# Bergvca/string_grouper

Hardware: AMD Instinct MI355X
Metric: hot-path rows/sec (the device path of match_strings: tokenise + tf-idf + postings + SpGEMM-topn, inputs resident in HBM), 663k-name self-join ntop=10 min_sim=0.8; match_strings end to end: match_strings_rows_per_s (higher is better)
Workload: dtype f32

## Files before the change

### string_grouper_amd/csrc/sg_postings.hip

```cpp
#include <stdlib.h>

#include <memory>
#include <optional>

#include "sg_internal.h"
#include "sg_scan.h"

__device__ __forceinline__ int64_t row_of_thread(int64_t g, int32_t tile_log2, int32_t n_tiles) {
    return ((g % n_tiles) << tile_log2) | (g / n_tiles);
}

template <typename T>
__global__ void __launch_bounds__(256) postings_count(const int64_t *__restrict__ indptr,
                                                      const int32_t *__restrict__ indices, int64_t n_rows,
                                                      int32_t tile_log2, int32_t n_tiles, uint32_t *seg_counts) {
    const int64_t j = row_of_thread((int64_t)blockIdx.x * blockDim.x + threadIdx.x, tile_log2, n_tiles);
    if (j >= n_rows) return;
    const int64_t lo = indptr[j], hi = indptr[j + 1];
    const uint32_t t = (uint32_t)(j >> tile_log2);
    for (int64_t p = lo; p < hi; ++p) {
        const int64_t bin = (int64_t)indices[p] * n_tiles + t;
        atomicAdd(&seg_counts[bin], 1u);
    }
}
// ... 66 lines not shown
                                                     uint32_t freq_min, float inv_norm_up, int32_t fold_log2) {
    const int64_t j = row_of_thread((int64_t)blockIdx.x * blockDim.x + threadIdx.x, tile_log2, n_tiles);
    if (j >= n_rows) return;
    const int64_t lo = indptr[j], hi = indptr[j + 1];
    const uint32_t t = (uint32_t)(j >> tile_log2);
    const uint32_t col = (uint32_t)(j & (((int64_t)1 << tile_log2) - 1));
    const float fq = out_filt ? frequent_norm_ratio<T>(indices, data, lo, hi, seg, n_tiles, freq_min, inv_norm_up) : 0.f;
    for (int64_t p = lo; p < hi; ++p) {
        const int64_t bin = (int64_t)indices[p] * n_tiles + t;
        const uint32_t pos = seg[bin] + atomicAdd(&cursor[bin], 1u);
        emit_posting<T>(out_rows, out_vals, out_filt, pos, col, data[p], fq, tile_log2, inv_norm_up, t, fold_log2);
    }
}

#define SG_POST_ROWS 4
__global__ void __launch_bounds__(1024) postings_count_lds(const int64_t *__restrict__ indptr,
                                                           const int32_t *__restrict__ indices, int64_t n_rows,
                                                           int32_t tile_log2, int32_t n_terms, int32_t split,
                                                           uint32_t *__restrict__ cnt ) {
    extern __shared__ uint32_t hist[];
    const int64_t t = blockIdx.x / split;
    const int32_t part = blockIdx.x % split;
    for (int k = threadIdx.x; k < n_terms; k += blockDim.x) hist[k] = 0;
    __syncthreads();
    const int64_t part_rows = ((int64_t)1 << tile_log2) / split;
    const int64_t j0 = (t << tile_log2) + part * part_rows;
    int64_t j1 = j0 + part_rows;
    if (j1 > n_rows) j1 = n_rows;
    const int sub = threadIdx.x & 15;
    const int64_t groups = blockDim.x >> 4;
    for (int64_t jb = j0 + (threadIdx.x >> 4) * SG_POST_ROWS; jb < j1; jb += groups * SG_POST_ROWS) {
        int64_t lo[SG_POST_ROWS], hi[SG_POST_ROWS];
#pragma unroll
        for (int r = 0; r < SG_POST_ROWS; ++r) {
            const bool valid = jb + r < j1;
            lo[r] = valid ? indptr[jb + r] : 0;
            hi[r] = valid ? indptr[jb + r + 1] : 0;
        }
        int32_t k0[SG_POST_ROWS];
#pragma unroll
        for (int r = 0; r < SG_POST_ROWS; ++r) k0[r] = lo[r] + sub < hi[r] ? indices[lo[r] + sub] : -1;
#pragma unroll
        for (int r = 0; r < SG_POST_ROWS; ++r) {
            if (k0[r] >= 0) atomicAdd(&hist[k0[r]], 1u);
            for (int64_t p = lo[r] + sub + 16; p < hi[r]; p += 16) atomicAdd(&hist[indices[p]], 1u);
        }
    }
    __syncthreads();
    uint32_t *mine = cnt + (int64_t)blockIdx.x * n_terms;
    for (int k = threadIdx.x; k < n_terms; k += blockDim.x) mine[k] = hist[k];
}

__global__ void __launch_bounds__(1024) postings_colscan_kernel(uint32_t *__restrict__ cnt, int32_t n_wgs, int32_t n_terms,
                                                                uint32_t freq_min, uint32_t *__restrict__ term_len,
                                                                uint8_t *__restrict__ is_frequent) {
    __shared__ uint32_t part_sum[16][64];
    const int kk = threadIdx.x & 63, c = threadIdx.x >> 6;
    const int64_t k = (int64_t)blockIdx.x * 64 + kk;
    const int32_t run = (n_wgs + 15) / 16;
    const int32_t w0 = c * run, w1 = min(w0 + run, n_wgs);
    uint32_t s = 0;
    if (k < n_terms)
        for (int32_t w = w0; w < w1; ++w) s += cnt[(int64_t)w * n_terms + k];
    part_sum[c][kk] = s;
    __syncthreads();
// ... 73 lines not shown
                                                          const uint32_t *__restrict__ term_start,
                                                          const uint8_t *__restrict__ is_frequent, int32_t *out_rows,
                                                          T *out_vals, uint32_t *out_filt, float inv_norm_up, int32_t fold_log2) {
    extern __shared__ uint32_t cursor[];
    uint32_t *freq_bits = cursor + n_terms;
    const int64_t t = blockIdx.x / split;
    const int32_t part = blockIdx.x % split;
    for (int k = threadIdx.x; k < (n_terms + 31) / 32; k += blockDim.x) freq_bits[k] = 0;
    const uint32_t *mine = cnt + (int64_t)blockIdx.x * n_terms;
    for (int k = threadIdx.x; k < n_terms; k += blockDim.x) cursor[k] = term_start[k] + mine[k];
    __syncthreads();
    if (out_filt)
        for (int k = threadIdx.x; k < n_terms; k += blockDim.x)
            if (is_frequent[k]) atomicOr(&freq_bits[k >> 5], 1u << (k & 31));
    __syncthreads();
    const int64_t part_rows = ((int64_t)1 << tile_log2) / split;
    const int64_t j0 = (t << tile_log2) + part * part_rows;
    int64_t j1 = j0 + part_rows;
    if (j1 > n_rows) j1 = n_rows;
    const int lane = threadIdx.x & 63, sub = lane & 15;
    (void)lane;
    const int64_t groups = blockDim.x >> 4;
    const int64_t trips = (j1 - j0 + groups * SG_POST_ROWS - 1) / (groups * SG_POST_ROWS);
    for (int64_t it = 0; it < trips; ++it) {
        const int64_t jb = j0 + (it * groups + (threadIdx.x >> 4)) * SG_POST_ROWS;
        int64_t lo[SG_POST_ROWS], hi[SG_POST_ROWS];
#pragma unroll
        for (int r = 0; r < SG_POST_ROWS; ++r) {
            const bool valid = jb + r < j1;
            lo[r] = valid ? indptr[jb + r] : 0;
            hi[r] = valid ? indptr[jb + r + 1] : 0;
        }
        int32_t k0[SG_POST_ROWS];
// ... 39 lines not shown
#endif
#if defined(SG_K3_PROBE_NO_STORE)
                if (pos == 0xFFFFFFF0u)
#endif
                emit_posting<T>(out_rows, out_vals, out_filt, pos, col, v0[r], fq[r], tile_log2, inv_norm_up, (uint32_t)t, fold_log2);
            }
            for (int64_t p = lo[r] + sub + 16; p < hi[r]; p += 16) {
                const uint32_t pos = atomicAdd(&cursor[indices[p]], 1u);
                emit_posting<T>(out_rows, out_vals, out_filt, pos, col, data[p], fq[r], tile_log2, inv_norm_up, (uint32_t)t, fold_log2);
            }
        }
    }
}

__device__ __forceinline__ uint32_t lds_get16(const uint32_t *w, uint32_t k) { return (w[k >> 1] >> ((k & 1u) << 4)) & 0xffffu; }
template <typename T>
__global__ void __launch_bounds__(1024) postings_fill_staged(const int64_t *__restrict__ indptr, const int32_t *__restrict__ indices,
                                                             const T *__restrict__ data, int64_t n_rows, int32_t tile_log2,
                                                             int32_t n_terms, int32_t split, int32_t chunk_rows, uint32_t stage_cap,
                                                             uint32_t *cnt , const uint32_t *__restrict__ term_start,
                                                             const uint8_t *__restrict__ is_frequent, uint32_t *__restrict__ out_filt,
                                                             float inv_norm_up, int32_t fold_log2) {
    extern __shared__ uint32_t lds[];
    const uint32_t w16 = ((uint32_t)n_terms + 1u) >> 1;
    uint32_t *lcnt = lds;
    uint32_t *freq_bits = lcnt + ((w16 + 3u) & ~3u);
    float *fqrow = reinterpret_cast<float *>(freq_bits + (((uint32_t)n_terms + 31u) >> 5));
    uint32_t *wave_tot = reinterpret_cast<uint32_t *>(fqrow + chunk_rows);
    uint32_t *stage = wave_tot + 32;
    const int64_t t = blockIdx.x / split;
    const int32_t part = blockIdx.x % split;
    uint32_t *mine = cnt + (int64_t)blockIdx.x * n_terms;
    for (uint32_t k = threadIdx.x; k < (((uint32_t)n_terms + 31u) >> 5); k += blockDim.x) freq_bits[k] = 0;
    __syncthreads();
    for (int k = threadIdx.x; k < n_terms; k += blockDim.x)
        if (is_frequent[k]) atomicOr(&freq_bits[k >> 5], 1u << (k & 31));
    __syncthreads();
    const int64_t part_rows = ((int64_t)1 << tile_log2) / split;
    const int64_t j0 = (t << tile_log2) + part * part_rows;
    int64_t j1 = j0 + part_rows;
    if (j1 > n_rows) j1 = n_rows;
    const int lane = threadIdx.x & 63, sub = lane & 15, wave = threadIdx.x >> 6;
    const int64_t groups = blockDim.x >> 4;
    const uint32_t last_k = (uint32_t)n_terms - 1u;
    bool any_big = false;
    for (int64_t c0 = j0; c0 < j1; c0 += chunk_rows) {
        const int64_t c1 = c0 + chunk_rows < j1 ? c0 + chunk_rows : j1;
        const int64_t e = indptr[c1] - indptr[c0];
        any_big = any_big || e > (int64_t)stage_cap || e > 65535;
    }
    for (int64_t c0 = j0; c0 < j1; c0 += chunk_rows) {
        const int64_t c1 = c0 + chunk_rows < j1 ? c0 + chunk_rows : j1;
        const int64_t trips = (c1 - c0 + groups * SG_POST_ROWS - 1) / (groups * SG_POST_ROWS);
        if (any_big) {
            for (int64_t it = 0; it < trips; ++it) {
                const int64_t jb = c0 + (it * groups + (threadIdx.x >> 4)) * SG_POST_ROWS;
#pragma unroll
                for (int r = 0; r < SG_POST_ROWS; ++r) {
                    const bool valid = jb + r < c1;
                    const int64_t lo = valid ? indptr[jb + r] : 0, hi = valid ? indptr[jb + r + 1] : 0;
                    double f2 = 0.0;
                    for (int64_t p = lo + sub; p < hi; p += 16) {
                        const int32_t k = indices[p];
                        if ((freq_bits[k >> 5] >> (k & 31)) & 1u) f2 += (double)data[p] * (double)data[p];
                    }
#pragma unroll
                    for (int d = 8; d > 0; d >>= 1) {
                        const uint64_t bits = (uint64_t)__double_as_longlong(f2);
                        const uint32_t l = (uint32_t)__shfl_xor((int)(uint32_t)bits, d, 64), h = (uint32_t)__shfl_xor((int)(uint32_t)(bits >> 32), d, 64);
                        f2 += __longlong_as_double((long long)(((uint64_t)h << 32) | l));
                    }
                    const float fq = frequent_norm_ratio_of(f2, inv_norm_up);
                    const uint32_t col = (uint32_t)(jb + r - (t << tile_log2));
                    for (int64_t p = lo + sub; p < hi; p += 16) {
                        const int32_t k = indices[p];
                        const uint32_t pos = term_start[k] + atomicAdd(&mine[k], 1u);
                        out_filt[pos] = filter_posting(col, (float)data[p], fq, tile_log2, inv_norm_up, (uint32_t)t, fold_log2);
                    }
                }
            }
            __syncthreads();
            continue;
        }
        for (uint32_t w = threadIdx.x; w < w16; w += blockDim.x) lcnt[w] = 0;
        __syncthreads();
        for (int64_t it = 0; it < trips; ++it) {
            const int64_t jb = c0 + (it * groups + (threadIdx.x >> 4)) * SG_POST_ROWS;
            int64_t lo[SG_POST_ROWS], hi[SG_POST_ROWS];
#pragma unroll
            for (int r = 0; r < SG_POST_ROWS; ++r) {
                const bool valid = jb + r < c1;
                lo[r] = valid ? indptr[jb + r] : 0;
                hi[r] = valid ? indptr[jb + r + 1] : 0;
            }
            int32_t k0[SG_POST_ROWS];
            T v0[SG_POST_ROWS];
#pragma unroll
            for (int r = 0; r < SG_POST_ROWS; ++r) {
                const bool have = lo[r] + sub < hi[r];
                k0[r] = have ? indices[lo[r] + sub] : -1;
                v0[r] = have ? data[lo[r] + sub] : (T)0;
            }
#pragma unroll
            for (int r = 0; r < SG_POST_ROWS; ++r) {
                double f2 = 0.0;
                if (k0[r] >= 0) {
                    atomicAdd(&lcnt[(uint32_t)k0[r] >> 1], 1u << (((uint32_t)k0[r] & 1u) << 4));
                    if ((freq_bits[k0[r] >> 5] >> (k0[r] & 31)) & 1u) f2 = (double)v0[r] * (double)v0[r];
                }
                for (int64_t p = lo[r] + sub + 16; p < hi[r]; p += 16) {
                    const int32_t k = indices[p];
                    atomicAdd(&lcnt[(uint32_t)k >> 1], 1u << (((uint32_t)k & 1u) << 4));
                    if ((freq_bits[k >> 5] >> (k & 31)) & 1u) f2 += (double)data[p] * (double)data[p];
                }
#pragma unroll
                for (int d = 8; d > 0; d >>= 1) {
                    const uint64_t bits = (uint64_t)__double_as_longlong(f2);
                    const uint32_t l = (uint32_t)__shfl_xor((int)(uint32_t)bits, d, 64), h = (uint32_t)__shfl_xor((int)(uint32_t)(bits >> 32), d, 64);
                    f2 += __longlong_as_double((long long)(((uint64_t)h << 32) | l));
                }
                if (sub == 0 && jb + r < c1) fqrow[jb + r - c0] = frequent_norm_ratio_of(f2, inv_norm_up);
            }
        }
        __syncthreads();
        {
            const uint32_t per = (w16 + blockDim.x - 1u) / blockDim.x;
            const uint32_t wa = threadIdx.x * per, wb = wa + per < w16 ? wa + per : w16;
            uint32_t sum = 0;
            for (uint32_t w = wa; w < wb; ++w) sum += (lcnt[w] & 0xffffu) + (lcnt[w] >> 16);
            uint32_t tot;
            uint32_t run = block_exclusive_scan<uint32_t>(sum, wave_tot, &tot);
            for (uint32_t w = wa; w < wb; ++w) {
                const uint32_t c = lcnt[w];
                const uint32_t a = run;
                run += c & 0xffffu;
                const uint32_t b = run;
                run += c >> 16;
                lcnt[w] = a | (b << 16);
            }
        }
        __syncthreads();
        for (int64_t it = 0; it < trips; ++it) {
            const int64_t jb = c0 + (it * groups + (threadIdx.x >> 4)) * SG_POST_ROWS;
            int64_t lo[SG_POST_ROWS], hi[SG_POST_ROWS];
#pragma unroll
            for (int r = 0; r < SG_POST_ROWS; ++r) {
                const bool valid = jb + r < c1;
                lo[r] = valid ? indptr[jb + r] : 0;
                hi[r] = valid ? indptr[jb + r + 1] : 0;
            }
            int32_t k0[SG_POST_ROWS];
            T v0[SG_POST_ROWS];
#pragma unroll
            for (int r = 0; r < SG_POST_ROWS; ++r) {
                const bool have = lo[r] + sub < hi[r];
                k0[r] = have ? indices[lo[r] + sub] : -1;
                v0[r] = have ? data[lo[r] + sub] : (T)0;
            }
#pragma unroll
            for (int r = 0; r < SG_POST_ROWS; ++r) {
                const float fq = jb + r < c1 ? fqrow[jb + r - c0] : 0.f;
                const uint32_t col = (uint32_t)(jb + r - (t << tile_log2));
                if (k0[r] >= 0) {
                    const uint32_t sh = ((uint32_t)k0[r] & 1u) << 4;
                    const uint32_t pos = (atomicAdd(&lcnt[(uint32_t)k0[r] >> 1], 1u << sh) >> sh) & 0xffffu;
                    stage[pos] = filter_posting(col, (float)v0[r], fq, tile_log2, inv_norm_up, (uint32_t)t, fold_log2);
                }
                for (int64_t p = lo[r] + sub + 16; p < hi[r]; p += 16) {
                    const uint32_t k = (uint32_t)indices[p];
                    const uint32_t sh = (k & 1u) << 4;
                    const uint32_t pos = (atomicAdd(&lcnt[k >> 1], 1u << sh) >> sh) & 0xffffu;
                    stage[pos] = filter_posting(col, (float)data[p], fq, tile_log2, inv_norm_up, (uint32_t)t, fold_log2);
                }
            }
        }
        __syncthreads();
        {
            constexpr int FB = 8;
            const uint32_t n_tg = ((uint32_t)n_terms + 63u) >> 6, waves = (uint32_t)(blockDim.x >> 6);
            for (uint32_t tg0 = (uint32_t)wave; tg0 < n_tg; tg0 += waves * FB) {
                uint32_t end_k[FB], start_k[FB], before[FB], G[FB];
                bool mine_has[FB];
#pragma unroll
                for (int b = 0; b < FB; ++b) {
                    const uint32_t tg = tg0 + (uint32_t)b * waves;
                    const uint32_t k = tg * 64u + (uint32_t)lane;
                    const bool live = tg < n_tg;
                    const uint32_t kc = k < last_k ? k : last_k;
                    end_k[b] = live ? lds_get16(lcnt, kc) : 0u;
                    start_k[b] = (!live || k == 0u) ? 0u : lds_get16(lcnt, (k - 1u) < last_k ? k - 1u : last_k);
                    mine_has[b] = live && k <= last_k && end_k[b] > start_k[b];
                }
#pragma unroll
                for (int b = 0; b < FB; ++b) {
                    const uint32_t k = (tg0 + (uint32_t)b * waves) * 64u + (uint32_t)lane;
                    before[b] = mine_has[b] ? mine[k] : 0u;
                    G[b] = mine_has[b] ? term_start[k] : 0u;
                }
#pragma unroll
                for (int b = 0; b < FB; ++b) {
                    const uint32_t tg = tg0 + (uint32_t)b * waves;
                    if (tg >= n_tg) break;
                    const uint32_t k = tg * 64u + (uint32_t)lane;
                    G[b] += before[b];
                    const uint32_t S = (uint32_t)__builtin_amdgcn_readlane((int)start_k[b], 0);
                    const uint32_t Eg = (uint32_t)__builtin_amdgcn_readlane((int)end_k[b], 63);
                    for (uint32_t e0 = S; e0 < Eg; e0 += 64u) {
                        const uint32_t e = e0 + (uint32_t)lane;
                        uint32_t lo = 0u, hi = 63u;
#pragma unroll
                        for (int step = 0; step < 6; ++step) {
                            const uint32_t mid = (lo + hi) >> 1;
                            const uint32_t km = tg * 64u + mid;
                            const bool right = lds_get16(lcnt, km < last_k ? km : last_k) > e;
                            hi = right ? mid : hi;
                            lo = right ? lo : mid + 1u;
                        }
                        const uint32_t tsel = lo < 63u ? lo : 63u;
                        const uint32_t kt = tg * 64u + tsel;
                        const uint32_t start_t = kt == 0u ? 0u : lds_get16(lcnt, (kt - 1u) < last_k ? kt - 1u : last_k);
                        const uint32_t G_t = (uint32_t)__shfl((int)G[b], (int)tsel, 64);
                        if (e < Eg) out_filt[G_t + (e - start_t)] = stage[e];
                    }
                    if (mine_has[b]) mine[k] = before[b] + (end_k[b] - start_k[b]);
                }
            }
        }
        __syncthreads();
    }
}

__global__ void __launch_bounds__(256) term_len_kernel(const uint32_t *__restrict__ seg, int64_t n_terms, int32_t n_tiles,
                                                       uint32_t *__restrict__ term_len) {
    const int64_t k = (int64_t)blockIdx.x * blockDim.x + threadIdx.x;
    if (k < n_terms) term_len[k] = seg[(k + 1) * n_tiles] - seg[k * n_tiles];
}

template <typename T>
__global__ void __launch_bounds__(256) fwd_pack(const int64_t *__restrict__ indptr, const int32_t *__restrict__ indices,
                                                const T *__restrict__ data, int64_t n_rows, int64_t nnz,
                                                const uint32_t *__restrict__ orig_of ,
                                                uint32_t *__restrict__ fwd_ptr , void *__restrict__ fwd) {
    const int64_t i = (int64_t)blockIdx.x * blockDim.x + threadIdx.x;
// ... 284 lines not shown
struct BuildPlan {
    bool cosine_like = false;
    float max_norm2 = 0.f;
    int32_t tile_cols = 0, tile_log2 = 0;
    int64_t n_tiles = 0, n_bins = 0;
    bool want_pruned = false, will_filter = false, want_q8 = false, want_blk = false;
    bool permute = false;
    bool early_rows = false;
    bool lds_path = false, lazy_full = false;
    int32_t fold_log2 = 0, nt_pad = 0, nv_pad = 0;
    float norm_up = 0.f;
    uint32_t freq_min = 0;
    bool staged = false;
    int32_t chunk_rows = 0;
    uint32_t stage_cap = 0;
    size_t staged_lds = 0;
    int32_t split = 1;
};

static int plan_build(sg_ctx *ctx, const sg_csr *B, int32_t tile_cols, int32_t flags, bool cosine_like, float max_norm2,
                      BuildPlan *out) {
    BuildPlan pl;
    pl.cosine_like = cosine_like;
    pl.max_norm2 = max_norm2;
    pl.want_pruned = cosine_like && !ctx->opt_is("SG_PRUNE", '0') && !(flags & SG_POSTINGS_EXACT_ONLY);
    if (tile_cols == 0) {
        tile_cols = B->dtype == SG_F64 ? 1024 : 2048;
        if (pl.want_pruned) {
            tile_cols = 4096;
            if (flags & SG_POSTINGS_TILE_FORM) tile_cols = 2048;
            else if (const char *v = ctx->opt("SG_PRUNE_TILE")) tile_cols = atoi(v) == 13 ? 8192 : (atoi(v) == 11 ? 2048 : 4096);
        }
    }
// ... 32 lines not shown
    if (const char *e = ctx->opt("SG_POSTINGS_LDS")) pl.lds_path = pl.lds_path && e[0] != '0';
    pl.lazy_full = pl.will_filter && pl.lds_path && !ctx->opt_is("SG_POSTINGS_LAZY", '0');
    if (pl.will_filter) {
        pl.nt_pad = (int32_t)((pl.n_tiles + 3) & ~(int64_t)3);
        if (pl.tile_log2 == 12 && !ctx->opt_is("SG_K4_STREAM", '0')) pl.fold_log2 = 3;
        if (pl.fold_log2 > 0) {
            const int64_t n_super = (pl.n_tiles + ((int64_t)1 << pl.fold_log2) - 1) >> pl.fold_log2;
            pl.nv_pad = (int32_t)((n_super + 3) & ~(int64_t)3);
        }
        double frac = 0.005;
        if (const char *v = ctx->opt("SG_PRUNE_FREQ")) frac = atof(v);
        const double fm = frac * (double)B->n_rows;
        pl.freq_min = fm < 1.0 ? 1u : (uint32_t)fm;
    }
    if (pl.lds_path) {
        pl.staged = pl.lazy_full && !ctx->opt_is("SG_FILL_STAGED", '0');
        const double mean_nnz = B->n_rows > 0 ? (double)B->nnz / (double)B->n_rows : 1.0;
        if (pl.staged) {
            const size_t fixed0 = ((((size_t)B->n_cols + 1) / 2 + 3) & ~(size_t)3) * 4 + (((size_t)B->n_cols + 31) / 32) * 4 + 32 * 4;
            pl.chunk_rows = 2048;
            for (;;) {
                const size_t fixed = fixed0 + (size_t)pl.chunk_rows * 4;
                const size_t room = fixed + 16384 < 158 * 1024 ? 158 * 1024 - fixed : 0;
                pl.stage_cap = (uint32_t)(room / 4);
                if (pl.stage_cap > 65535u) pl.stage_cap = 65535u;
                if ((double)pl.chunk_rows * mean_nnz * 1.2 + 64.0 <= (double)pl.stage_cap || pl.chunk_rows <= 64) break;
                pl.chunk_rows >>= 1;
            }
            pl.staged = (double)pl.chunk_rows * mean_nnz * 1.2 + 64.0 <= (double)pl.stage_cap;
            pl.staged_lds = fixed0 + (size_t)pl.chunk_rows * 4 + (size_t)pl.stage_cap * 4;
            if (const char *v = ctx->opt("SG_FILL_STAGE_CAP"))
                if (atoi(v) > 0 && (uint32_t)atoi(v) < pl.stage_cap) pl.stage_cap = (uint32_t)atoi(v);
        }
        int32_t split = 1;
        while (split < 4 && pl.n_tiles * split < ctx->num_cu && (tile_cols / (split * 2)) >= 1024 &&
               (pl.n_bins * split * 2 + 1) < ((int64_t)1 << 31))
            split *= 2;
        if (pl.staged)
            while (split < 8 && pl.n_tiles * split < 2 * (int64_t)ctx->num_cu && (tile_cols / (split * 2)) >= 512 &&
                   (pl.n_bins * split * 2 + 1) < ((int64_t)1 << 31))
                split *= 2;
        if (const char *e = ctx->opt("SG_POSTINGS_SPLIT")) {
            const int o = atoi(e);
            if ((o == 1 || o == 2 || o == 4) && tile_cols / o >= 64 && pl.n_bins * o + 1 < ((int64_t)1 << 31)) split = o;
        }
        pl.split = split;
    }
    *out = pl;
    return SG_OK;
}

struct EarlyRows {
    void *fwd = nullptr;
    uint32_t *fwd_ptr = nullptr;
    void *q8 = nullptr;
    bool written = false;
};

static int alloc_early_rows(Scratch &early, const sg_csr *B, const BuildPlan &plan, EarlyRows *rows) {
// ... 135 lines not shown
        SG_TRY(sg_alloc(ctx, 2 * ((size_t)B->n_rows + 2), &p->d_fwd_ptr));
        if (plan.want_q8 && !p->d_blk) SG_TRY(ctx->alloc((size_t)SG_Q8_STRIDE * ((size_t)B->n_rows + 1), &p->d_q8));
    }
    SG_TRY(sg_alloc(ctx, (size_t)B->nnz + 512, &p->d_filt));
    p->nt_pad = plan.nt_pad;
    SG_TRY(sg_alloc(ctx, (size_t)(B->n_cols + 1) * (size_t)p->nt_pad + 4, &p->d_ends));
    p->fold_log2 = plan.fold_log2;
    p->nv_pad = plan.nv_pad;
    if (p->fold_log2 > 0) SG_TRY(sg_alloc(ctx, (size_t)(B->n_cols + 1) * (size_t)p->nv_pad + 4, &p->d_ends8));
    p->norm_up = plan.norm_up;
    p->freq_min = plan.freq_min;
    return SG_OK;
}

static int lds_count_scan_fill(sg_ctx *ctx, sg_postings *p, uint32_t *cnt ,
                               uint32_t *term_len, uint8_t *is_frequent, bool values_only, bool fill) {
    const sg_csr *B = &p->src;
    const int32_t split = p->split > 0 ? p->split : 1;
    const int64_t wgs64 = (int64_t)p->n_tiles * split;
    const unsigned wgs = (unsigned)wgs64;
    const size_t lds = lds_counter_bytes(B->n_cols);
    uint32_t *filt = values_only ? nullptr : p->d_filt;
    const float inv_norm = filt ? 1.0f / p->norm_up : 0.f;
    const int32_t fold_log2 = values_only ? 0 : p->fold_log2;
    SG_TRY(allow_dynamic_lds<postings_count_lds>(124 * 1024));
    hipLaunchKernelGGL(postings_count_lds, dim3(wgs), dim3(1024), (size_t)B->n_cols * 4, ctx->stream, B->d_indptr, B->d_indices,
                       B->n_rows, p->tile_log2, (int32_t)B->n_cols, split, cnt);
    hipLaunchKernelGGL(postings_colscan_kernel, dim3((unsigned)((B->n_cols + 63) / 64)), dim3(1024), 0, ctx->stream, cnt,
                       (int32_t)wgs64, (int32_t)B->n_cols, values_only ? 0u : p->freq_min, term_len, is_frequent);
    if (!values_only) SG_TRY(sg_exclusive_scan_u32(ctx, term_len, p->d_term_start, B->n_cols, p->d_term_start + B->n_cols));
    if (fill)
        SG_TRY(by_dtype(B->dtype, [&](auto tag) -> int {
            using T = decltype(tag);
            constexpr auto kern = postings_fill_lds<T>;
            SG_TRY(allow_dynamic_lds<kern>(124 * 1024));
            hipLaunchKernelGGL(kern, dim3(wgs), dim3(1024), lds, ctx->stream, B->d_indptr, B->d_indices,
                               (const T *)B->d_data, B->n_rows, p->tile_log2, (int32_t)B->n_cols, split, (const uint32_t *)cnt,
                               (const uint32_t *)p->d_term_start, (const uint8_t *)is_frequent, p->d_rows, (T *)p->d_vals, filt,
                               inv_norm, fold_log2);
            return SG_OK;
        }));
    return hipGetLastError() == hipSuccess ? SG_OK : SG_ERR_HIP;
}

static int fill_lds_path(sg_ctx *ctx, sg_postings *p, const BuildPlan &plan) {
    const sg_csr *B = &p->src;
    const unsigned wgs = (unsigned)((int64_t)p->n_tiles * plan.split);
    Scratch scratch(ctx);
    uint32_t *cnt = nullptr;
    uint8_t *is_frequent = nullptr;
    SG_TRY(scratch.alloc((size_t)((int64_t)p->n_tiles * plan.split * B->n_cols) + 1, &cnt));
    SG_TRY(scratch.alloc((size_t)B->n_cols + 4, &is_frequent));
    SG_TRY(sg_alloc(ctx, (size_t)B->n_cols + 2, &p->d_term_start));
    SG_TRY(lds_count_scan_fill(ctx, p, cnt, p->d_term_len, is_frequent, false, !plan.staged));
    if (p->d_fwd_ptr) SG_TRY(ctx->alloc(256, (void **)&p->d_score_ctx));
    hipLaunchKernelGGL(postings_tables_kernel, dim3((unsigned)((B->n_cols + 64) / 64)), dim3(1024), 0, ctx->stream, (const uint32_t *)cnt,
                       (const uint32_t *)p->d_term_start, (int32_t)B->n_cols, p->n_tiles, plan.split, p->d_seg, p->d_ends,
                       p->nt_pad, p->d_ends8, p->nv_pad, p->fold_log2, score_ctx_of(p), p->d_score_ctx,
                       p->d_filt ? p->d_filt + B->nnz : (uint32_t *)nullptr);
    if (plan.staged)
        SG_TRY(by_dtype(B->dtype, [&](auto tag) -> int {
            using T = decltype(tag);
            constexpr auto kern = postings_fill_staged<T>;
            SG_TRY(allow_dynamic_lds<kern>(160 * 1024));
            hipLaunchKernelGGL(kern, dim3(wgs), dim3(1024), plan.staged_lds, ctx->stream, B->d_indptr,
                               B->d_indices, (const T *)B->d_data, B->n_rows, p->tile_log2, (int32_t)B->n_cols, plan.split,
                               plan.chunk_rows, plan.stage_cap, cnt, (const uint32_t *)p->d_term_start, (const uint8_t *)is_frequent,
                               p->d_filt, 1.0f / p->norm_up, p->fold_log2);
            return SG_OK;
        }));
    return hipGetLastError() == hipSuccess ? SG_OK : SG_ERR_HIP;
}

static int fill_global_path(sg_ctx *ctx, sg_postings *p, const BuildPlan &plan) {
    const sg_csr *B = &p->src;
    const int64_t n_bins = plan.n_bins;
    const unsigned grid = (unsigned)((((int64_t)p->n_tiles << p->tile_log2) + 255) / 256);
    const float inv_norm = p->d_filt ? 1.0f / p->norm_up : 0.f;
    Scratch scratch(ctx);
    uint32_t *cursor = nullptr;
    SG_TRY(scratch.alloc((size_t)n_bins + 1, &cursor));
    SG_HIP_TRY(hipMemsetAsync(p->d_seg, 0, sizeof(uint32_t) * (size_t)(n_bins + 1), ctx->stream));
// ... 158 lines not shown
int sg_postings_ensure_full(sg_ctx *ctx, const sg_postings *cp) {
    sg_postings *p = const_cast<sg_postings *>(cp);
    if (p->d_vals || p->nnz <= 0) return SG_OK;
    const sg_csr *B = &p->src;
    Scratch scratch(ctx);
    uint32_t *cnt = nullptr, *len_scratch = nullptr;
    if (B->dtype == SG_F64) SG_TRY(scratch.alloc((size_t)B->nnz + 64, &p->d_rows));
    int st = scratch.alloc_bytes(((size_t)B->nnz + 64) * 8, &p->d_vals);
    if (st == SG_OK && !p->d_term_start) {
        sg_set_error("postings were built without the LDS path: nothing is lazy there");
        st = SG_ERR_BADARG;
    }
    const int32_t split = p->split > 0 ? p->split : 1;
    if (st == SG_OK) st = scratch.alloc((size_t)((int64_t)p->n_tiles * split * B->n_cols) + 1, &cnt);
    if (st == SG_OK) st = scratch.alloc((size_t)B->n_cols + 2, &len_scratch);
    if (st == SG_OK) st = lds_count_scan_fill(ctx, p, cnt, len_scratch, nullptr, true, true);
    if (st != SG_OK) {
        p->d_vals = nullptr;
        p->d_rows = nullptr;
        return st;
    }
    scratch.keep(p->d_rows);
    scratch.keep(p->d_vals);
    return SG_OK;
}

extern "C" int sg_postings_free(sg_postings *p) {
    if (!p) return SG_OK;
    p->ctx->release(p->d_seg);
    p->ctx->release(p->d_term_len);
    p->ctx->release(p->d_term_start);
// ... 21 lines not shown
```

Measured before the change: 107.2 million.

## Reuse count histograms in staged postings fill and pick split via cost model

```diff
diff --git a/string_grouper_amd/csrc/sg_postings.hip b/string_grouper_amd/csrc/sg_postings.hip
--- a/string_grouper_amd/csrc/sg_postings.hip
+++ b/string_grouper_amd/csrc/sg_postings.hip
@@ -104,18 +104,21 @@
 }
 
 #define SG_POST_ROWS 4
+__host__ __device__ __forceinline__ int64_t part_begin(int32_t part, int32_t split, int32_t tile_log2) {
+    return part >= split ? (int64_t)1 << tile_log2 : ((((int64_t)part << tile_log2) / split) & ~(int64_t)63);
+}
 __global__ void __launch_bounds__(1024) postings_count_lds(const int64_t *__restrict__ indptr,
                                                            const int32_t *__restrict__ indices, int64_t n_rows,
                                                            int32_t tile_log2, int32_t n_terms, int32_t split,
-                                                           uint32_t *__restrict__ cnt ) {
+                                                           uint32_t *__restrict__ cnt ,
+                                                           uint32_t *__restrict__ cnt16 ) {
     extern __shared__ uint32_t hist[];
     const int64_t t = blockIdx.x / split;
     const int32_t part = blockIdx.x % split;
     for (int k = threadIdx.x; k < n_terms; k += blockDim.x) hist[k] = 0;
     __syncthreads();
-    const int64_t part_rows = ((int64_t)1 << tile_log2) / split;
-    const int64_t j0 = (t << tile_log2) + part * part_rows;
-    int64_t j1 = j0 + part_rows;
+    const int64_t j0 = (t << tile_log2) + part_begin(part, split, tile_log2);
+    int64_t j1 = (t << tile_log2) + part_begin(part + 1, split, tile_log2);
     if (j1 > n_rows) j1 = n_rows;
     const int sub = threadIdx.x & 15;
     const int64_t groups = blockDim.x >> 4;
@@ -127,18 +130,30 @@
             lo[r] = valid ? indptr[jb + r] : 0;
             hi[r] = valid ? indptr[jb + r + 1] : 0;
         }
-        int32_t k0[SG_POST_ROWS];
-#pragma unroll
-        for (int r = 0; r < SG_POST_ROWS; ++r) k0[r] = lo[r] + sub < hi[r] ? indices[lo[r] + sub] : -1;
+        int32_t k0[SG_POST_ROWS], k1[SG_POST_ROWS];
+#pragma unroll
+        for (int r = 0; r < SG_POST_ROWS; ++r) {
+            k0[r] = lo[r] + sub < hi[r] ? indices[lo[r] + sub] : -1;
+            k1[r] = lo[r] + sub + 16 < hi[r] ? indices[lo[r] + sub + 16] : -1;
+        }
 #pragma unroll
         for (int r = 0; r < SG_POST_ROWS; ++r) {
             if (k0[r] >= 0) atomicAdd(&hist[k0[r]], 1u);
-            for (int64_t p = lo[r] + sub + 16; p < hi[r]; p += 16) atomicAdd(&hist[indices[p]], 1u);
+            if (k1[r] >= 0) atomicAdd(&hist[k1[r]], 1u);
+            for (int64_t p = lo[r] + sub + 32; p < hi[r]; p += 16) atomicAdd(&hist[indices[p]], 1u);
         }
     }
     __syncthreads();
     uint32_t *mine = cnt + (int64_t)blockIdx.x * n_terms;
     for (int k = threadIdx.x; k < n_terms; k += blockDim.x) mine[k] = hist[k];
+    if (cnt16) {
+        const int w16 = (n_terms + 1) >> 1;
+        uint32_t *mine16 = cnt16 + (int64_t)blockIdx.x * w16;
+        for (int w = threadIdx.x; w < w16; w += blockDim.x) {
+            const uint32_t a = hist[2 * w], b = 2 * w + 1 < n_terms ? hist[2 * w + 1] : 0u;
+            mine16[w] = (a < 0xffffu ? a : 0xffffu) | ((b < 0xffffu ? b : 0xffffu) << 16);
+        }
+    }
 }
 
 __global__ void __launch_bounds__(1024) postings_colscan_kernel(uint32_t *__restrict__ cnt, int32_t n_wgs, int32_t n_terms,
@@ -242,9 +257,8 @@
         for (int k = threadIdx.x; k < n_terms; k += blockDim.x)
             if (is_frequent[k]) atomicOr(&freq_bits[k >> 5], 1u << (k & 31));
     __syncthreads();
-    const int64_t part_rows = ((int64_t)1 << tile_log2) / split;
-    const int64_t j0 = (t << tile_log2) + part * part_rows;
-    int64_t j1 = j0 + part_rows;
+    const int64_t j0 = (t << tile_log2) + part_begin(part, split, tile_log2);
+    int64_t j1 = (t << tile_log2) + part_begin(part + 1, split, tile_log2);
     if (j1 > n_rows) j1 = n_rows;
     const int lane = threadIdx.x & 63, sub = lane & 15;
     (void)lane;
@@ -314,41 +328,71 @@
 }
 
 __device__ __forceinline__ uint32_t lds_get16(const uint32_t *w, uint32_t k) { return (w[k >> 1] >> ((k & 1u) << 4)) & 0xffffu; }
+__host__ __device__ __forceinline__ uint32_t staged_rowp_words(int32_t chunk_rows) { return ((uint32_t)chunk_rows + 4u) & ~3u; }
 template <typename T>
 __global__ void __launch_bounds__(1024) postings_fill_staged(const int64_t *__restrict__ indptr, const int32_t *__restrict__ indices,
                                                              const T *__restrict__ data, int64_t n_rows, int32_t tile_log2,
                                                              int32_t n_terms, int32_t split, int32_t chunk_rows, uint32_t stage_cap,
-                                                             uint32_t *cnt , const uint32_t *__restrict__ term_start,
+                                                             uint32_t stage_alloc ,
+                                                             uint32_t *cnt ,
+                                                             const uint32_t *__restrict__ cnt16 ,
+                                                             const uint32_t *__restrict__ term_start,
                                                              const uint8_t *__restrict__ is_frequent, uint32_t *__restrict__ out_filt,
                                                              float inv_norm_up, int32_t fold_log2) {
     extern __shared__ uint32_t lds[];
     const uint32_t w16 = ((uint32_t)n_terms + 1u) >> 1;
     uint32_t *lcnt = lds;
     uint32_t *freq_bits = lcnt + ((w16 + 3u) & ~3u);
-    float *fqrow = reinterpret_cast<float *>(freq_bits + (((uint32_t)n_terms + 31u) >> 5));
-    uint32_t *wave_tot = reinterpret_cast<uint32_t *>(fqrow + chunk_rows);
-    uint32_t *stage = wave_tot + 32;
+    uint32_t *wave_tot = freq_bits + (((uint32_t)n_terms + 31u) >> 5);
+    uint32_t *rowp = wave_tot + 32;
+    uint32_t *stage = rowp + staged_rowp_words(chunk_rows);
+    uint16_t *sterm = reinterpret_cast<uint16_t *>(stage + stage_alloc);
     const int64_t t = blockIdx.x / split;
     const int32_t part = blockIdx.x % split;
     uint32_t *mine = cnt + (int64_t)blockIdx.x * n_terms;
-    for (uint32_t k = threadIdx.x; k < (((uint32_t)n_terms + 31u) >> 5); k += blockDim.x) freq_bits[k] = 0;
-    __syncthreads();
-    for (int k = threadIdx.x; k < n_terms; k += blockDim.x)
-        if (is_frequent[k]) atomicOr(&freq_bits[k >> 5], 1u << (k & 31));
-    __syncthreads();
-    const int64_t part_rows = ((int64_t)1 << tile_log2) / split;
-    const int64_t j0 = (t << tile_log2) + part * part_rows;
-    int64_t j1 = j0 + part_rows;
+    const int64_t j0 = (t << tile_log2) + part_begin(part, split, tile_log2);
+    int64_t j1 = (t << tile_log2) + part_begin(part + 1, split, tile_log2);
     if (j1 > n_rows) j1 = n_rows;
+    if (j1 <= j0) return;
     const int lane = threadIdx.x & 63, sub = lane & 15, wave = threadIdx.x >> 6;
     const int64_t groups = blockDim.x >> 4;
-    const uint32_t last_k = (uint32_t)n_terms - 1u;
     bool any_big = false;
     for (int64_t c0 = j0; c0 < j1; c0 += chunk_rows) {
         const int64_t c1 = c0 + chunk_rows < j1 ? c0 + chunk_rows : j1;
         const int64_t e = indptr[c1] - indptr[c0];
         any_big = any_big || e > (int64_t)stage_cap || e > 65535;
     }
+    const bool one_chunk = j1 - j0 <= chunk_rows && !any_big;
+    {
+        const uint32_t *flags4 = reinterpret_cast<const uint32_t *>(is_frequent);
+        for (uint32_t w = threadIdx.x; w < (((uint32_t)n_terms + 31u) >> 5); w += blockDim.x) {
+            uint32_t f[8];
+#pragma unroll
+            for (uint32_t q = 0; q < 8; ++q) f[q] = (w * 8u + q) * 4u < (uint32_t)n_terms ? flags4[w * 8u + q] : 0u;
+            uint32_t bits = 0;
+#pragma unroll
+            for (uint32_t i = 0; i < 32; ++i)
+                if (w * 32u + i < (uint32_t)n_terms && ((f[i >> 2] >> ((i & 3u) << 3)) & 0xffu)) bits |= 1u << i;
+            freq_bits[w] = bits;
+        }
+    }
+    auto load_row_pointers = [&](int64_t c0, int64_t c1) {
+        const int64_t base = indptr[c0];
+        for (int64_t i = threadIdx.x; i <= c1 - c0; i += blockDim.x) rowp[i] = (uint32_t)(indptr[c0 + i] - base);
+    };
+    if (one_chunk) {
+        const uint32_t *mine16 = cnt16 + (int64_t)blockIdx.x * w16;
+        for (uint32_t w0 = threadIdx.x; w0 < w16; w0 += blockDim.x * 8u) {
+            uint32_t v[8];
+#pragma unroll
+            for (uint32_t q = 0; q < 8; ++q) v[q] = w0 + q * blockDim.x < w16 ? mine16[w0 + q * blockDim.x] : 0u;
+#pragma unroll
+            for (uint32_t q = 0; q < 8; ++q)
+                if (w0 + q * blockDim.x < w16) lcnt[w0 + q * blockDim.x] = v[q];
+        }
+        load_row_pointers(j0, j1);
+    }
+    __syncthreads();
     for (int64_t c0 = j0; c0 < j1; c0 += chunk_rows) {
         const int64_t c1 = c0 + chunk_rows < j1 ? c0 + chunk_rows : j1;
         const int64_t trips = (c1 - c0 + groups * SG_POST_ROWS - 1) / (groups * SG_POST_ROWS);
@@ -379,56 +423,46 @@
                     }
                 }
             }
+            continue;
+        }
+        const int64_t chunk_base = indptr[c0];
+        if (!one_chunk) {
+            for (uint32_t w = threadIdx.x; w < w16; w += blockDim.x) lcnt[w] = 0;
+            load_row_pointers(c0, c1);
             __syncthreads();
-            continue;
-        }
-        for (uint32_t w = threadIdx.x; w < w16; w += blockDim.x) lcnt[w] = 0;
-        __syncthreads();
-        for (int64_t it = 0; it < trips; ++it) {
-            const int64_t jb = c0 + (it * groups + (threadIdx.x >> 4)) * SG_POST_ROWS;
-            int64_t lo[SG_POST_ROWS], hi[SG_POST_ROWS];
-#pragma unroll
-            for (int r = 0; r < SG_POST_ROWS; ++r) {
-                const bool valid = jb + r < c1;
-                lo[r] = valid ? indptr[jb + r] : 0;
-                hi[r] = valid ? indptr[jb + r + 1] : 0;
+            for (int64_t it = 0; it < trips; ++it) {
+                const int64_t jb = c0 + (it * groups + (threadIdx.x >> 4)) * SG_POST_ROWS;
+                int64_t lo[SG_POST_ROWS], hi[SG_POST_ROWS];
+#pragma unroll
+                for (int r = 0; r < SG_POST_ROWS; ++r) {
+                    const bool valid = jb + r < c1;
+                    lo[r] = valid ? chunk_base + rowp[jb + r - c0] : 0;
+                    hi[r] = valid ? chunk_base + rowp[jb + r - c0 + 1] : 0;
+                }
+                int32_t k0[SG_POST_ROWS], k1[SG_POST_ROWS];
+#pragma unroll
+                for (int r = 0; r < SG_POST_ROWS; ++r) {
+                    k0[r] = lo[r] + sub < hi[r] ? indices[lo[r] + sub] : -1;
+                    k1[r] = lo[r] + sub + 16 < hi[r] ? indices[lo[r] + sub + 16] : -1;
+                }
+#pragma unroll
+                for (int r = 0; r < SG_POST_ROWS; ++r) {
+                    if (k0[r] >= 0) atomicAdd(&lcnt[(uint32_t)k0[r] >> 1], 1u << (((uint32_t)k0[r] & 1u) << 4));
+                    if (k1[r] >= 0) atomicAdd(&lcnt[(uint32_t)k1[r] >> 1], 1u << (((uint32_t)k1[r] & 1u) << 4));
+                    for (int64_t p = lo[r] + sub + 32; p < hi[r]; p += 16) {
+                        const uint32_t k = (uint32_t)indices[p];
+                        atomicAdd(&lcnt[k >> 1], 1u << ((k & 1u) << 4));
+                    }
+                }
             }
-            int32_t k0[SG_POST_ROWS];
-            T v0[SG_POST_ROWS];
-#pragma unroll
-            for (int r = 0; r < SG_POST_ROWS; ++r) {
-                const bool have = lo[r] + sub < hi[r];
-                k0[r] = have ? indices[lo[r] + sub] : -1;
-                v0[r] = have ? data[lo[r] + sub] : (T)0;
-            }
-#pragma unroll
-            for (int r = 0; r < SG_POST_ROWS; ++r) {
-                double f2 = 0.0;
-                if (k0[r] >= 0) {
-                    atomicAdd(&lcnt[(uint32_t)k0[r] >> 1], 1u << (((uint32_t)k0[r] & 1u) << 4));
-                    if ((freq_bits[k0[r] >> 5] >> (k0[r] & 31)) & 1u) f2 = (double)v0[r] * (double)v0[r];
-                }
-                for (int64_t p = lo[r] + sub + 16; p < hi[r]; p += 16) {
-                    const int32_t k = indices[p];
-                    atomicAdd(&lcnt[(uint32_t)k >> 1], 1u << (((uint32_t)k & 1u) << 4));
-                    if ((freq_bits[k >> 5] >> (k & 31)) & 1u) f2 += (double)data[p] * (double)data[p];
-                }
-#pragma unroll
-                for (int d = 8; d > 0; d >>= 1) {
-                    const uint64_t bits = (uint64_t)__double_as_longlong(f2);
-                    const uint32_t l = (uint32_t)__shfl_xor((int)(uint32_t)bits, d, 64), h = (uint32_t)__shfl_xor((int)(uint32_t)(bits >> 32), d, 64);
-                    f2 += __longlong_as_double((long long)(((uint64_t)h << 32) | l));
-                }
-                if (sub == 0 && jb + r < c1) fqrow[jb + r - c0] = frequent_norm_ratio_of(f2, inv_norm_up);
-            }
-        }
-        __syncthreads();
+            __syncthreads();
+        }
+        uint32_t tot;
         {
             const uint32_t per = (w16 + blockDim.x - 1u) / blockDim.x;
-            const uint32_t wa = threadIdx.x * per, wb = wa + per < w16 ? wa + per : w16;
+            const uint32_t wa = threadIdx.x * per < w16 ? threadIdx.x * per : w16, wb = wa + per < w16 ? wa + per : w16;
             uint32_t sum = 0;
             for (uint32_t w = wa; w < wb; ++w) sum += (lcnt[w] & 0xffffu) + (lcnt[w] >> 16);
-            uint32_t tot;
             uint32_t run = block_exclusive_scan<uint32_t>(sum, wave_tot, &tot);
             for (uint32_t w = wa; w < wb; ++w) {
                 const uint32_t c = lcnt[w];
@@ -446,87 +480,95 @@
 #pragma unroll
             for (int r = 0; r < SG_POST_ROWS; ++r) {
                 const bool valid = jb + r < c1;
-                lo[r] = valid ? indptr[jb + r] : 0;
-                hi[r] = valid ? indptr[jb + r + 1] : 0;
+                lo[r] = valid ? chunk_base + rowp[jb + r - c0] : 0;
+                hi[r] = valid ? chunk_base + rowp[jb + r - c0 + 1] : 0;
             }
-            int32_t k0[SG_POST_ROWS];
-            T v0[SG_POST_ROWS];
+            int32_t k0[SG_POST_ROWS], k1[SG_POST_ROWS];
+            T v0[SG_POST_ROWS], v1[SG_POST_ROWS];
 #pragma unroll
             for (int r = 0; r < SG_POST_ROWS; ++r) {
-                const bool have = lo[r] + sub < hi[r];
+                const bool have = lo[r] + sub < hi[r], more = lo[r] + sub + 16 < hi[r];
                 k0[r] = have ? indices[lo[r] + sub] : -1;
                 v0[r] = have ? data[lo[r] + sub] : (T)0;
+                k1[r] = more ? indices[lo[r] + sub + 16] : -1;
+                v1[r] = more ? data[lo[r] + sub + 16] : (T)0;
             }
 #pragma unroll
             for (int r = 0; r < SG_POST_ROWS; ++r) {
-                const float fq = jb + r < c1 ? fqrow[jb + r - c0] : 0.f;
+                double f2 = 0.0;
+                if (k0[r] >= 0 && ((freq_bits[k0[r] >> 5] >> (k0[r] & 31)) & 1u)) f2 = (double)v0[r] * (double)v0[r];
+                if (k1[r] >= 0 && ((freq_bits[k1[r] >> 5] >> (k1[r] & 31)) & 1u)) f2 += (double)v1[r] * (double)v1[r];
+                for (int64_t p = lo[r] + sub + 32; p < hi[r]; p += 16) {
+                    const int32_t k = indices[p];
+                    if ((freq_bits[k >> 5] >> (k & 31)) & 1u) f2 += (double)data[p] * (double)data[p];
+                }
+#pragma unroll
+                for (int d = 8; d > 0; d >>= 1) {
+                    const uint64_t bits = (uint64_t)__double_as_longlong(f2);
+                    const uint32_t l = (uint32_t)__shfl_xor((int)(uint32_t)bits, d, 64), h = (uint32_t)__shfl_xor((int)(uint32_t)(bits >> 32), d, 64);
+                    f2 += __longlong_as_double((long long)(((uint64_t)h << 32) | l));
+                }
+                const float fq = frequent_norm_ratio_of(f2, inv_norm_up);
                 const uint32_t col = (uint32_t)(jb + r - (t << tile_log2));
                 if (k0[r] >= 0) {
                     const uint32_t sh = ((uint32_t)k0[r] & 1u) << 4;
                     const uint32_t pos = (atomicAdd(&lcnt[(uint32_t)k0[r] >> 1], 1u << sh) >> sh) & 0xffffu;
                     stage[pos] = filter_posting(col, (float)v0[r], fq, tile_log2, inv_norm_up, (uint32_t)t, fold_log2);
+                    sterm[pos] = (uint16_t)k0[r];
                 }
-                for (int64_t p = lo[r] + sub + 16; p < hi[r]; p += 16) {
+                if (k1[r] >= 0) {
+                    const uint32_t sh = ((uint32_t)k1[r] & 1u) << 4;
+                    const uint32_t pos = (atomicAdd(&lcnt[(uint32_t)k1[r] >> 1], 1u << sh) >> sh) & 0xffffu;
+                    stage[pos] = filter_posting(col, (float)v1[r], fq, tile_log2, inv_norm_up, (uint32_t)t, fold_log2);
+                    sterm[pos] = (uint16_t)k1[r];
+                }
+                for (int64_t p = lo[r] + sub + 32; p < hi[r]; p += 16) {
                     const uint32_t k = (uint32_t)indices[p];
                     const uint32_t sh = (k & 1u) << 4;
                     const uint32_t pos = (atomicAdd(&lcnt[k >> 1], 1u << sh) >> sh) & 0xffffu;
                     stage[pos] = filter_posting(col, (float)data[p], fq, tile_log2, inv_norm_up, (uint32_t)t, fold_log2);
+                    sterm[pos] = (uint16_t)k;
                 }
             }
         }
         __syncthreads();
         {
             constexpr int FB = 8;
-            const uint32_t n_tg = ((uint32_t)n_terms + 63u) >> 6, waves = (uint32_t)(blockDim.x >> 6);
-            for (uint32_t tg0 = (uint32_t)wave; tg0 < n_tg; tg0 += waves * FB) {
-                uint32_t end_k[FB], start_k[FB], before[FB], G[FB];
-                bool mine_has[FB];
+            const uint32_t stride = (uint32_t)blockDim.x;
+            for (uint32_t e0 = (uint32_t)wave * 64u; e0 < tot; e0 += stride * FB) {
+                uint32_t delta[FB];
+                bool head[FB];
 #pragma unroll
                 for (int b = 0; b < FB; ++b) {
-                    const uint32_t tg = tg0 + (uint32_t)b * waves;
-                    const uint32_t k = tg * 64u + (uint32_t)lane;
-                    const bool live = tg < n_tg;
-                    const uint32_t kc = k < last_k ? k : last_k;
-                    end_k[b] = live ? lds_get16(lcnt, kc) : 0u;
-                    start_k[b] = (!live || k == 0u) ? 0u : lds_get16(lcnt, (k - 1u) < last_k ? k - 1u : last_k);
-                    mine_has[b] = live && k <= last_k && end_k[b] > start_k[b];
+                    const uint32_t e = e0 + (uint32_t)b * stride + (uint32_t)lane;
+                    const uint32_t k = e < tot ? (uint32_t)sterm[e] : 0xffffffffu;
+                    const uint32_t before = (uint32_t)__shfl_up((int)k, 1, 64);
+                    head[b] = e < tot && (lane == 0 || k != before);
+                    delta[b] = 0u;
+                    if (head[b]) {
+                        const uint32_t start = k == 0u ? 0u : lds_get16(lcnt, k - 1u);
+                        delta[b] = term_start[k] + mine[k] - start;
+                    }
                 }
 #pragma unroll
                 for (int b = 0; b < FB; ++b) {
-                    const uint32_t k = (tg0 + (uint32_t)b * waves) * 64u + (uint32_t)lane;
-                    before[b] = mine_has[b] ? mine[k] : 0u;
-                    G[b] = mine_has[b] ? term_start[k] : 0u;
-                }
-#pragma unroll
-                for (int b = 0; b < FB; ++b) {
-                    const uint32_t tg = tg0 + (uint32_t)b * waves;
-                    if (tg >= n_tg) break;
-                    const uint32_t k = tg * 64u + (uint32_t)lane;
-                    G[b] += before[b];
-                    const uint32_t S = (uint32_t)__builtin_amdgcn_readlane((int)start_k[b], 0);
-                    const uint32_t Eg = (uint32_t)__builtin_amdgcn_readlane((int)end_k[b], 63);
-                    for (uint32_t e0 = S; e0 < Eg; e0 += 64u) {
-                        const uint32_t e = e0 + (uint32_t)lane;
-                        uint32_t lo = 0u, hi = 63u;
-#pragma unroll
-                        for (int step = 0; step < 6; ++step) {
-                            const uint32_t mid = (lo + hi) >> 1;
-                            const uint32_t km = tg * 64u + mid;
-                            const bool right = lds_get16(lcnt, km < last_k ? km : last_k) > e;
-                            hi = right ? mid : hi;
-                            lo = right ? lo : mid + 1u;
-                        }
-                        const uint32_t tsel = lo < 63u ? lo : 63u;
-                        const uint32_t kt = tg * 64u + tsel;
-                        const uint32_t start_t = kt == 0u ? 0u : lds_get16(lcnt, (kt - 1u) < last_k ? kt - 1u : last_k);
-                        const uint32_t G_t = (uint32_t)__shfl((int)G[b], (int)tsel, 64);
-                        if (e < Eg) out_filt[G_t + (e - start_t)] = stage[e];
-                    }
-                    if (mine_has[b]) mine[k] = before[b] + (end_k[b] - start_k[b]);
+                    const uint32_t e = e0 + (uint32_t)b * stride + (uint32_t)lane;
+                    const uint64_t heads = __ballot(head[b]) & (~0ull >> (63 - lane));
+                    const int src = heads ? 63 - __builtin_clzll(heads) : 0;
+                    const uint32_t d = (uint32_t)__shfl((int)delta[b], src, 64);
+                    if (e < tot) out_filt[d + e] = stage[e];
                 }
             }
         }
         __syncthreads();
+        if (!one_chunk) {
+            for (uint32_t e = threadIdx.x; e < tot; e += blockDim.x) {
+                const uint32_t k = (uint32_t)sterm[e];
+                const uint32_t start = k == 0u ? 0u : lds_get16(lcnt, k - 1u);
+                if (e == start) mine[k] += lds_get16(lcnt, k) - start;
+            }
+            __syncthreads();
+        }
     }
 }
 
@@ -841,9 +883,53 @@
     bool staged = false;
     int32_t chunk_rows = 0;
     uint32_t stage_cap = 0;
+    uint32_t stage_alloc = 0;
     size_t staged_lds = 0;
     int32_t split = 1;
 };
+
+struct SplitCost {
+    int32_t split = 1;
+    int64_t parts = 0, part_rows = 0, chunks = 0, fill_rounds = 0;
+    double fill_us = 0, table_us = 0, total_us = 0;
+};
+static constexpr double SG_SPLIT_US_PER_TERM_AND_CHUNK = 0.78e-3, SG_SPLIT_US_PER_POSTING = 2.9e-3, SG_SPLIT_US_PER_POSTING_RECOUNT = 0.53e-3,
+                        SG_SPLIT_US_PER_CELL = 3.7e-6;
+static constexpr int32_t SG_SPLIT_MAX = 16, SG_SPLIT_MIN_PART_ROWS = 512;
+static SplitCost split_cost(int32_t split, int32_t tile_log2, int64_t n_tiles, int64_t n_terms, double mean_nnz, int32_t chunk_rows,
+                            int32_t num_cu) {
+    SplitCost c;
+    c.split = split;
+    c.parts = n_tiles * split;
+    for (int32_t part = 0; part < split; ++part) {
+        const int64_t rows = part_begin(part + 1, split, tile_log2) - part_begin(part, split, tile_log2);
+        if (rows > c.part_rows) c.part_rows = rows;
+    }
+    const int64_t cus = num_cu > 0 ? num_cu : 1;
+    c.fill_rounds = (c.parts + cus - 1) / cus;
+    c.chunks = (c.part_rows + chunk_rows - 1) / chunk_rows;
+    const double postings = (double)c.part_rows * mean_nnz;
+    c.fill_us = (double)c.fill_rounds * ((double)c.chunks * SG_SPLIT_US_PER_TERM_AND_CHUNK * (double)n_terms +
+                                         (SG_SPLIT_US_PER_POSTING + (c.chunks > 1 ? SG_SPLIT_US_PER_POSTING_RECOUNT : 0.0)) * postings);
+    c.table_us = SG_SPLIT_US_PER_CELL * (double)c.parts * (double)n_terms;
+    c.total_us = c.fill_us + c.table_us;
+    return c;
+}
+static int32_t choose_split(sg_ctx *ctx, const BuildPlan &pl, int64_t n_terms, double mean_nnz) {
+    SplitCost best;
+    const bool say = ctx->opt_is("SG_POSTINGS_PLAN", '1');
+    for (int32_t s = 1; s <= SG_SPLIT_MAX; ++s) {
+        if (s > 1 && (pl.tile_cols / s < SG_SPLIT_MIN_PART_ROWS || pl.n_bins * s + 1 >= ((int64_t)1 << 31))) break;
+        const SplitCost c = split_cost(s, pl.tile_log2, pl.n_tiles, n_terms, mean_nnz, pl.chunk_rows, ctx->num_cu);
+        if (say)
+            fprintf(stderr, "sg postings plan: split %d: %lld parts of <= %lld rows (%lld chunks), %lld rounds of the fill, us fill %.1f table %.1f = %.1f\n",
+                    s, (long long)c.parts, (long long)c.part_rows, (long long)c.chunks, (long long)c.fill_rounds, c.fill_us, c.table_us, c.total_us);
+        if (s == 1 || c.total_us < best.total_us) best = c;
+    }
+    if (say) fprintf(stderr, "sg postings plan: chosen split %d (%lld tiles, %lld terms, chunks of %d rows)\n", best.split, (long long)pl.n_tiles,
+                     (long long)n_terms, pl.chunk_rows);
+    return best.split;
+}
 
 static int plan_build(sg_ctx *ctx, const sg_csr *B, int32_t tile_cols, int32_t flags, bool cosine_like, float max_norm2,
                       BuildPlan *out) {
@@ -906,35 +992,34 @@
         pl.freq_min = fm < 1.0 ? 1u : (uint32_t)fm;
     }
     if (pl.lds_path) {
-        pl.staged = pl.lazy_full && !ctx->opt_is("SG_FILL_STAGED", '0');
+        pl.staged = pl.lazy_full && !ctx->opt_is("SG_FILL_STAGED", '0') && B->n_cols <= 65535;
         const double mean_nnz = B->n_rows > 0 ? (double)B->nnz / (double)B->n_rows : 1.0;
         if (pl.staged) {
             const size_t fixed0 = ((((size_t)B->n_cols + 1) / 2 + 3) & ~(size_t)3) * 4 + (((size_t)B->n_cols + 31) / 32) * 4 + 32 * 4;
-            pl.chunk_rows = 2048;
-            for (;;) {
-                const size_t fixed = fixed0 + (size_t)pl.chunk_rows * 4;
-                const size_t room = fixed + 16384 < 158 * 1024 ? 158 * 1024 - fixed : 0;
-                pl.stage_cap = (uint32_t)(room / 4);
-                if (pl.stage_cap > 65535u) pl.stage_cap = 65535u;
-                if ((double)pl.chunk_rows * mean_nnz * 1.2 + 64.0 <= (double)pl.stage_cap || pl.chunk_rows <= 64) break;
-                pl.chunk_rows >>= 1;
-            }
-            pl.staged = (double)pl.chunk_rows * mean_nnz * 1.2 + 64.0 <= (double)pl.stage_cap;
-            pl.staged_lds = fixed0 + (size_t)pl.chunk_rows * 4 + (size_t)pl.stage_cap * 4;
+            const size_t room = fixed0 + 16384 < 158 * 1024 ? 158 * 1024 - fixed0 : 0;
+            const double per_row = (mean_nnz * 1.2 > 1.0 ? mean_nnz * 1.2 : 1.0) * 6.0 + 4.0;
+            const double fit = ((double)room - 64.0 * 6.0 - 32.0) / per_row;
+            pl.chunk_rows = fit >= 2048.0 ? 2048 : (fit > 0.0 ? (int32_t)fit & ~63 : 0);
+            pl.staged = pl.chunk_rows >= 64;
+            const size_t rowp_bytes = (size_t)staged_rowp_words(pl.chunk_rows) * 4;
+            pl.stage_alloc = pl.staged ? (uint32_t)((room - rowp_bytes) / 6) & ~1u : 0u;
+            if (pl.stage_alloc > 65534u) pl.stage_alloc = 65534u;
+            pl.stage_cap = pl.stage_alloc;
+            pl.staged_lds = fixed0 + rowp_bytes + (size_t)pl.stage_alloc * 6;
             if (const char *v = ctx->opt("SG_FILL_STAGE_CAP"))
                 if (atoi(v) > 0 && (uint32_t)atoi(v) < pl.stage_cap) pl.stage_cap = (uint32_t)atoi(v);
         }
         int32_t split = 1;
-        while (split < 4 && pl.n_tiles * split < ctx->num_cu && (tile_cols / (split * 2)) >= 1024 &&
-               (pl.n_bins * split * 2 + 1) < ((int64_t)1 << 31))
-            split *= 2;
-        if (pl.staged)
-            while (split < 8 && pl.n_tiles * split < 2 * (int64_t)ctx->num_cu && (tile_cols / (split * 2)) >= 512 &&
+        if (pl.staged) {
+            split = choose_split(ctx, pl, B->n_cols, mean_nnz);
+        } else {
+            while (split < 4 && pl.n_tiles * split < ctx->num_cu && (tile_cols / (split * 2)) >= 1024 &&
                    (pl.n_bins * split * 2 + 1) < ((int64_t)1 << 31))
                 split *= 2;
+        }
         if (const char *e = ctx->opt("SG_POSTINGS_SPLIT")) {
             const int o = atoi(e);
-            if ((o == 1 || o == 2 || o == 4) && tile_cols / o >= 64 && pl.n_bins * o + 1 < ((int64_t)1 << 31)) split = o;
+            if (o >= 1 && o <= SG_SPLIT_MAX && tile_cols / o >= 64 && pl.n_bins * o + 1 < ((int64_t)1 << 31)) split = o;
         }
         pl.split = split;
     }
@@ -1100,6 +1185,7 @@
 }
 
 static int lds_count_scan_fill(sg_ctx *ctx, sg_postings *p, uint32_t *cnt ,
+                               uint32_t *cnt16 ,
                                uint32_t *term_len, uint8_t *is_frequent, bool values_only, bool fill) {
     const sg_csr *B = &p->src;
     const int32_t split = p->split > 0 ? p->split : 1;
@@ -1111,7 +1197,7 @@
     const int32_t fold_log2 = values_only ? 0 : p->fold_log2;
     SG_TRY(allow_dynamic_lds<postings_count_lds>(124 * 1024));
     hipLaunchKernelGGL(postings_count_lds, dim3(wgs), dim3(1024), (size_t)B->n_cols * 4, ctx->stream, B->d_indptr, B->d_indices,
-                       B->n_rows, p->tile_log2, (int32_t)B->n_cols, split, cnt);
+                       B->n_rows, p->tile_log2, (int32_t)B->n_cols, split, cnt, cnt16);
     hipLaunchKernelGGL(postings_colscan_kernel, dim3((unsigned)((B->n_cols + 63) / 64)), dim3(1024), 0, ctx->stream, cnt,
                        (int32_t)wgs64, (int32_t)B->n_cols, values_only ? 0u : p->freq_min, term_len, is_frequent);
     if (!values_only) SG_TRY(sg_exclusive_scan_u32(ctx, term_len, p->d_term_start, B->n_cols, p->d_term_start + B->n_cols));
@@ -1133,12 +1219,13 @@
     const sg_csr *B = &p->src;
     const unsigned wgs = (unsigned)((int64_t)p->n_tiles * plan.split);
     Scratch scratch(ctx);
-    uint32_t *cnt = nullptr;
+    uint32_t *cnt = nullptr, *cnt16 = nullptr;
     uint8_t *is_frequent = nullptr;
     SG_TRY(scratch.alloc((size_t)((int64_t)p->n_tiles * plan.split * B->n_cols) + 1, &cnt));
+    if (plan.staged) SG_TRY(scratch.alloc((size_t)((int64_t)p->n_tiles * plan.split * ((B->n_cols + 1) / 2)) + 1, &cnt16));
     SG_TRY(scratch.alloc((size_t)B->n_cols + 4, &is_frequent));
     SG_TRY(sg_alloc(ctx, (size_t)B->n_cols + 2, &p->d_term_start));
-    SG_TRY(lds_count_scan_fill(ctx, p, cnt, p->d_term_len, is_frequent, false, !plan.staged));
+    SG_TRY(lds_count_scan_fill(ctx, p, cnt, cnt16, p->d_term_len, is_frequent, false, !plan.staged));
     if (p->d_fwd_ptr) SG_TRY(ctx->alloc(256, (void **)&p->d_score_ctx));
     hipLaunchKernelGGL(postings_tables_kernel, dim3((unsigned)((B->n_cols + 64) / 64)), dim3(1024), 0, ctx->stream, (const uint32_t *)cnt,
                        (const uint32_t *)p->d_term_start, (int32_t)B->n_cols, p->n_tiles, plan.split, p->d_seg, p->d_ends,
@@ -1151,7 +1238,8 @@
             SG_TRY(allow_dynamic_lds<kern>(160 * 1024));
             hipLaunchKernelGGL(kern, dim3(wgs), dim3(1024), plan.staged_lds, ctx->stream, B->d_indptr,
                                B->d_indices, (const T *)B->d_data, B->n_rows, p->tile_log2, (int32_t)B->n_cols, plan.split,
-                               plan.chunk_rows, plan.stage_cap, cnt, (const uint32_t *)p->d_term_start, (const uint8_t *)is_frequent,
+                               plan.chunk_rows, plan.stage_cap, plan.stage_alloc, cnt, (const uint32_t *)cnt16,
+                               (const uint32_t *)p->d_term_start, (const uint8_t *)is_frequent,
                                p->d_filt, 1.0f / p->norm_up, p->fold_log2);
             return SG_OK;
         }));
@@ -1340,7 +1428,7 @@
     const int32_t split = p->split > 0 ? p->split : 1;
     if (st == SG_OK) st = scratch.alloc((size_t)((int64_t)p->n_tiles * split * B->n_cols) + 1, &cnt);
     if (st == SG_OK) st = scratch.alloc((size_t)B->n_cols + 2, &len_scratch);
-    if (st == SG_OK) st = lds_count_scan_fill(ctx, p, cnt, len_scratch, nullptr, true, true);
+    if (st == SG_OK) st = lds_count_scan_fill(ctx, p, cnt, nullptr, len_scratch, nullptr, true, true);
     if (st != SG_OK) {
         p->d_vals = nullptr;
         p->d_rows = nullptr;
```

After: 109.3 million, median of 6. +1.9%, better.
